# openjamoses/TOSEM-2021-Replication

Measured on NVIDIA H100. Metric: source MB/s scanned (tokenise + line-hash + classify + aggregate), higher is better.
Workload: dtype u8

## Files before the change

tosem-2021-replication_b200/csrc/tsm_device.cuh:

```cuda
#pragma once
#include <cstdint>
#include <cuda_runtime.h>
#include "../../include/tosemscan.h"
#include "../../include/tsm_categories.h"

namespace tsm {

constexpr uint32_t CH = 4096;
constexpr uint32_t PRE = 16;
constexpr uint32_t EXT = 240;
constexpr uint32_t BUF = PRE + CH + EXT;
constexpr uint32_t STRIPE = BUF / 32;
static_assert(STRIPE * 32 == BUF && STRIPE % 8 == 0 && (STRIPE / 8) % 2 == 1, "stripe geometry");
constexpr uint32_t LUT_BYTES = 1024 + 128;

constexpr uint32_t B_FIRST = (1u << 0) | (1u << 6) | (1u << 13) | (1u << 18) | (1u << 21) | (1u << 25) | (1u << 29) | (1u << 30) | (1u << 31);
constexpr uint32_t AF_ASSERT = 1u << 5, AF_EXPECT = 1u << 12, A_CLASS = 1u << 17, A_DEF = 1u << 20, A_TEST = 1u << 24,
                   A_VOID = 1u << 28, A_BRACE = 1u << 29, B_F = 1u << 30;
constexpr uint32_t PY_G1 = A_DEF, PY_G2 = A_CLASS, CJ_G1 = A_TEST, CJ_G2 = A_BRACE | A_CLASS | A_VOID;

constexpr uint8_t LF_CAND = 1, LF_HDR = 2, LF_FIX = 4;

struct Ctrl {
  uint32_t n_cand;
  uint32_t n_hev;
  uint32_t n_aev;
  uint32_t overflow;
  uint32_t n_lh;
  uint32_t lh_overflow;
  uint32_t cls_done;
};

constexpr unsigned long long TSM_DIFF_TRACE_MAX_INTS = 1ull << 28;
constexpr long long TSM_DIFF_TRACE_MAX_D = 23168;
static_assert((TSM_DIFF_TRACE_MAX_D + 1) * (TSM_DIFF_TRACE_MAX_D + 2) / 2 <= (long long)TSM_DIFF_TRACE_MAX_INTS && (TSM_DIFF_TRACE_MAX_D + 2) * (TSM_DIFF_TRACE_MAX_D + 3) / 2 > (long long)TSM_DIFF_TRACE_MAX_INTS, "cap");

struct SlabCtl { uint32_t n_units, work; };

struct ScanParams {
  const uint8_t* arena;
  const int32_t* off;
  const int32_t* len;
  const uint8_t* ext;
  const uint16_t* grp;
  int32_t n_files;
  int32_t n_groups;
  uint32_t* unit_file;
  uint32_t* unit_begin;
  uint32_t unit_cap;
  SlabCtl* slab;
  int32_t f_begin, f_end;
  uint32_t unit_base;
  Ctrl* ctrl;
  tsm_file_stat* stats;
  unsigned long long* cand;
  uint32_t cand_cap;
  tsm_header_event* hev;
  uint32_t hev_cap;
  tsm_assert_event* aev;
  uint32_t aev_cap;
  unsigned long long* counts;
  uint32_t flags;
  unsigned long long* lh_hash;
  uint32_t* lh_end;
  uint8_t* lh_flag;
  uint32_t lh_cap;
  uint32_t* unit_lines;
  uint32_t* unit_out;
  uint32_t four;
  uint32_t cls_last;
};

constexpr unsigned long long M61 = 0x1FFFFFFFFFFFFFFFull;

__device__ __forceinline__ unsigned long long fold61(unsigned long long x) { return (x & M61) + (x >> 61); }
__device__ __forceinline__ unsigned long long rotl61(unsigned long long x, uint32_t r) {
  return ((x << r) & M61) | (x >> (61 - r));
}
__device__ __forceinline__ unsigned long long canon61(unsigned long long acc) {
  acc = fold61(fold61(acc));
  return acc == M61 ? 0ull : acc;
}
__device__ __forceinline__ unsigned long long mix_hash(unsigned long long h61, unsigned long long len) {
  unsigned long long x = h61 ^ (len * 0x9E3779B97F4A7C15ull);
  x ^= x >> 30; x *= 0xBF58476D1CE4E5B9ull;
  x ^= x >> 27; x *= 0x94D049BB133111EBull;
  x ^= x >> 31;
  return x;
}

__device__ __forceinline__ bool is_w(uint32_t c) { return c == 0x20 || c == 0x09 || c == 0x0D || c == 0x0B || c == 0x0C; }
__device__ __forceinline__ bool is_ident(uint32_t c) {
  return (c - 'a') < 26u || (c - 'A') < 26u || (c - '0') < 10u || c == '_';
}

__device__ __forceinline__ uint32_t smem_u32(const void* p) { return (uint32_t)__cvta_generic_to_shared(p); }
__device__ __forceinline__ void mbar_init(uint64_t* bar, uint32_t count) {
  asm volatile("mbarrier.init.shared::cta.b64 [%0], %1;" ::"r"(smem_u32(bar)), "r"(count));
}
__device__ __forceinline__ void fence_mbar_init() { asm volatile("fence.mbarrier_init.release.cluster;" ::: "memory"); }
__device__ __forceinline__ void fence_proxy_async() { asm volatile("fence.proxy.async.shared::cta;" ::: "memory"); }
__device__ __forceinline__ void mbar_expect_tx(uint64_t* bar, uint32_t bytes) {
  asm volatile("mbarrier.arrive.expect_tx.shared::cta.b64 _, [%0], %1;" ::"r"(smem_u32(bar)), "r"(bytes) : "memory");
}
__device__ __forceinline__ void bulk_load(void* dst, const void* src, uint32_t bytes, uint64_t* bar) {
  asm volatile("cp.async.bulk.shared::cluster.global.mbarrier::complete_tx::bytes [%0], [%1], %2, [%3];"
               ::"r"(smem_u32(dst)), "l"(src), "r"(bytes), "r"(smem_u32(bar)) : "memory");
}
__device__ __forceinline__ bool mbar_try_wait(uint64_t* bar, uint32_t parity) {
  uint32_t ok;
  asm volatile("{\n\t.reg .pred p;\n\tmbarrier.try_wait.parity.shared::cta.b64 p, [%1], %2;\n\tselp.u32 %0, 1, 0, p;\n\t}"
               : "=r"(ok) : "r"(smem_u32(bar)), "r"(parity) : "memory");
  return ok != 0;
}

}
```

tosem-2021-replication_b200/csrc/tsm_scan_kernels.cuh:

```cuda
#pragma once
#include "tsm_device.cuh"

namespace tsm {

__constant__ uint32_t c_lut[256];
__constant__ uint32_t c_lut_b[256];
__constant__ uint32_t c_elut[256];
__device__ uint8_t c_cat_slot[TSM_CAT_SLOTS];
__device__ uint16_t c_cat_off[TSM_CAT_NAMED + 1];
__device__ char c_cat_blob[TSM_CAT_BLOB_LEN + 1];

__global__ void k_plan(ScanParams p) {
  const int f = p.f_begin + blockIdx.x * blockDim.x + threadIdx.x;
  const int lane = threadIdx.x & 31;
  if (blockIdx.x == 0 && threadIdx.x == 0) p.ctrl->cls_done = p.ctrl->n_cand;
  uint32_t nu = 0;
  if (f < p.f_end) {
    nu = ((uint32_t)p.len[f] + CH - 1) / CH;
    if (nu != 1) p.stats[f] = tsm_file_stat{0, 0, 0, 0, 0};
  }
  uint32_t incl = nu;
#pragma unroll
  for (int d = 1; d < 32; d <<= 1) {
    uint32_t t = __shfl_up_sync(0xffffffffu, incl, d);
    if (lane >= d) incl += t;
  }
  const uint32_t total = __shfl_sync(0xffffffffu, incl, 31);
  uint32_t base = 0;
  if (lane == 31 && total) base = atomicAdd(&p.slab->n_units, total);
  base = __shfl_sync(0xffffffffu, base, 31);
  uint32_t at = p.unit_base + base + incl - nu;
  for (uint32_t u = 0; u < nu; ++u, ++at) {
    if (at < p.unit_cap) { p.unit_file[at] = (uint32_t)f; p.unit_begin[at] = u * CH; }
    else p.ctrl->overflow = 1;
  }
}

__device__ __forceinline__ uint32_t nl_word(uint32_t w) {
  const uint32_t y = w ^ 0x0A0A0A0Au;
  const uint32_t t = (y & 0x7F7F7F7Fu) + 0x7F7F7F7Fu;
  const uint32_t z = ~(t | y | 0x7F7F7F7Fu);
  return (z * 0x00204081u) >> 28;
}
__device__ __forceinline__ uint32_t spaces_of(unsigned long long w) {
  const unsigned long long x = w ^ 0x2020202020202020ull, k7 = 0x7F7F7F7F7F7F7F7Full;
  const unsigned long long nz = (((x & k7) + k7) | x) & ~k7;
  return nz ? ((uint32_t)__ffsll((long long)nz) - 1u) >> 3 : 8u;
}
struct SmemByte {
  const uint8_t* b;
  __device__ __forceinline__ uint32_t operator()(uint32_t i) const { return b[i]; }
  __device__ __forceinline__ unsigned long long load8(uint32_t i) const {
    const uint32_t a = i & ~7u, sh = 8u * (i & 7u);
    const unsigned long long lo = *reinterpret_cast<const unsigned long long*>(b + a);
    const unsigned long long hi = *reinterpret_cast<const unsigned long long*>(b + a + 8);
    return sh ? (lo >> sh) | (hi << (64u - sh)) : lo;
  }
  __device__ __forceinline__ uint32_t spaces8(uint32_t i) const { return spaces_of(load8(i)); }
};
struct HbmByte {
  const uint8_t* b;
  __device__ __forceinline__ uint32_t operator()(uint32_t i) const { return __ldg(b + i); }
  __device__ __forceinline__ unsigned long long load8(uint32_t i) const {
    const unsigned long long* w = reinterpret_cast<const unsigned long long*>(b) + (i >> 3);
    const uint32_t sh = 8u * (i & 7u);
    const unsigned long long lo = __ldg(w), hi = __ldg(w + 1);
    return sh ? (lo >> sh) | (hi << (64u - sh)) : lo;
  }
  __device__ __forceinline__ uint32_t spaces8(uint32_t i) const { return spaces_of(load8(i)); }
};
struct Accum { uint32_t lines, asserts, hdrs, fixes; unsigned long long digest; };

__device__ __forceinline__ uint32_t warp_reserve(uint32_t* counter, uint32_t n, int lane) {
  uint32_t base = 0;
  if (lane == 0 && n) base = atomicAdd(counter, n);
  return __shfl_sync(0xffffffffu, base, 0);
}

__device__ __forceinline__ const uint32_t* scan_lut() {
  extern __shared__ __align__(128) uint8_t smem[];
  return reinterpret_cast<const uint32_t*>(smem);
}

__device__ __forceinline__ void issue_load(const ScanParams& p, uint8_t* buf, uint64_t* bar, uint32_t fo,
                                           uint32_t size, uint32_t cb) {
  const uint32_t lb = cb ? cb - PRE : 0u;
  const uint32_t le = min(cb + CH + EXT, size);
  const uint32_t bytes = (le - lb + 15u) & ~15u;
  mbar_expect_tx(bar, bytes);
  bulk_load(buf + PRE - (cb - lb), p.arena + (size_t)fo + lb, bytes, bar);
}

struct Unit { uint32_t u, f, cb, fo, size; int ext; };

__device__ __forceinline__ Unit claim_unit(const ScanParams& p, uint32_t n_units, int lane) {
  Unit x{0, 0, 0, 0, 0, 0};
  if (lane == 0) x.u = atomicAdd(&p.slab->work, 1u);
  x.u = __shfl_sync(0xffffffffu, x.u, 0);
  if (x.u < n_units) {
    x.f = p.unit_file[p.unit_base + x.u];
    x.cb = p.unit_begin[p.unit_base + x.u];
    x.fo = (uint32_t)p.off[x.f];
    x.size = (uint32_t)p.len[x.f];
    x.ext = p.ext[x.f];
  }
  return x;
}

constexpr uint32_t CC_W = 1, CC_IDENT = 2, CC_STOP = 4;
constexpr uint32_t CLS_CAT_OFF_N = (TSM_CAT_NAMED + 2) & ~1u;
constexpr uint32_t CLS_CAT_WORDS = ((TSM_CAT_SLOTS + 2 * CLS_CAT_OFF_N + TSM_CAT_BLOB_LEN + 15) / 16) * 4;
constexpr uint32_t CLS_SMEM_BASE = 4 * (512 + CLS_CAT_WORDS + 4 * 1024 + 4);
constexpr uint32_t E_FIRST = (1u << 0) | (1u << 5) | (1u << 9) | (1u << 17) | (1u << 21) | (1u << 23) | (1u << 25) |
                             (1u << 27) | (1u << 29) | (1u << 30);

struct FileBytes {
  const unsigned long long* base; uint32_t cur_blk; unsigned long long w;
  uint32_t blk0; unsigned long long w0, w1, w2, w3;
  __device__ __forceinline__ FileBytes(const uint8_t* b, uint32_t first_byte)
      : base(reinterpret_cast<const unsigned long long*>(b)), cur_blk(0xFFFFFFFFu), w(0), blk0(first_byte >> 3) {
    w0 = __ldg(base + blk0); w1 = __ldg(base + blk0 + 1); w2 = __ldg(base + blk0 + 2); w3 = __ldg(base + blk0 + 3);
  }
  __device__ __forceinline__ unsigned long long word(uint32_t blk) const {
    const uint32_t d = blk - blk0;
    if (d < 4u) return d < 2u ? (d == 0u ? w0 : w1) : (d == 2u ? w2 : w3);
    return __ldg(base + blk);
  }
  __device__ __forceinline__ uint32_t get(uint32_t i) {
    const uint32_t blk = i >> 3;
    if (blk != cur_blk) { w = word(blk); cur_blk = blk; }
    return (uint32_t)(w >> (8u * (i & 7u))) & 0xFFu;
  }
  __device__ __forceinline__ unsigned long long get8(uint32_t i) const {
    const uint32_t blk = i >> 3, sh = 8u * (i & 7u);
    const unsigned long long lo = word(blk);
    if (sh == 0) return lo;
    return (lo >> sh) | (word(blk + 1) << (64u - sh));
  }
};

__device__ __forceinline__ unsigned long long low_bytes(unsigned long long v, uint32_t n) {
  return n >= 8 ? v : (v & ((1ull << (8u * n)) - 1ull));
}

__device__ __forceinline__ int stem_lookup(FileBytes& rd, uint32_t s, uint32_t n) {
  if (n < 2 || n > 9) return 0;
  const unsigned long long v = low_bytes(rd.get8(s), n);
  const uint32_t c9 = n == 9 ? rd.get(s + 8) : 0u;
  switch (n) {
    case 2:
      if (v == 0x5145ull) return 1;
      if (v == 0x454Eull) return 2;
      if (v == 0x5447ull) return 5;
      if (v == 0x4547ull) return 6;
      if (v == 0x544Cull) return 7;
      if (v == 0x454Cull) return 8;
      return 0;
    case 4:
      if (v == 0x45555254ull) return 3;
      if (v == 0x5241454Eull) return 9;
      return 0;
    case 5:
      if (v == 0x45534C4146ull) return 4;
      if (v == 0x574F524854ull) return 12;
      return 0;
    case 8: return v == 0x51455F54414F4C46ull ? 10 : 0;
    case 9: return (v == 0x455F454C42554F44ull && c9 == 'Q') ? 11 : 0;
    default: return 0;
  }
}

__device__ __forceinline__ int bare_assert_category(FileBytes& rd, uint32_t e0, uint32_t en, const uint32_t* elut, int deflt = 3,
                                                    bool not_prefix = true) {
  if (not_prefix && en >= 4 && (uint32_t)rd.get8(e0) == 0x20746F6Eu) return 2;
  uint32_t D = 0, A = 0;
  for (uint32_t a = 0; a < en; a += 8) {
    unsigned long long w = rd.get8(e0 + a);
    if (en - a < 8) w &= (1ull << (8u * (en - a))) - 1ull;
    const uint32_t lo = (uint32_t)w, hi = (uint32_t)(w >> 32);
#pragma unroll
    for (int k = 0; k < 4; ++k) { D = ((D + D) | E_FIRST) & elut[__byte_perm(lo, 0, 0x4440 + k)]; A |= D; }
#pragma unroll
    for (int k = 0; k < 4; ++k) { D = ((D + D) | E_FIRST) & elut[__byte_perm(hi, 0, 0x4440 + k)]; A |= D; }
  }
  if (((A & (1u << 4)) && (A & (1u << 8))) || (A & (1u << 16))) return 4;
  if (A & (1u << 20)) return 3;
  if (A & (1u << 22)) return 1;
  if (A & (1u << 24)) return 2;
  if (A & (1u << 26)) return 8;
  if (A & (1u << 28)) return 6;
  if (A & (1u << 29)) return 7;
  if (A & (1u << 30)) return 5;
  return deflt;
}

__device__ __noinline__ bool ident_eq(FileBytes& rd, uint32_t s, uint32_t n, const char* name, uint32_t len) {
  if (n != len) return false;
  for (uint32_t k = 0; k < len; ++k)
    if (rd.get(s + k) != (uint8_t)name[k]) return false;
  return true;
}

constexpr uint32_t BQ_CAP = 1024;

#ifndef TSM_CLS_MINB
#define TSM_CLS_MINB 1
#endif
template <bool REVB>
__global__ void __launch_bounds__(256, TSM_CLS_MINB) k_classify_t(ScanParams p) {
  extern __shared__ __align__(16) uint32_t csm[];
  uint32_t* cls = csm;
  uint32_t* elut = csm + 256;
  uint8_t* cat_slot = reinterpret_cast<uint8_t*>(csm + 512);
  uint16_t* cat_off = reinterpret_cast<uint16_t*>(cat_slot + TSM_CAT_SLOTS);
  uint8_t* cat_blob = reinterpret_cast<uint8_t*>(cat_off + CLS_CAT_OFF_N);
  uint4* bq = reinterpret_cast<uint4*>(csm + 512 + CLS_CAT_WORDS);
  uint32_t* bqn = csm + 512 + CLS_CAT_WORDS + 4 * BQ_CAP;
  uint32_t* hist = bqn + 4;
  const bool use_smem = p.n_groups <= 16;
  for (int i = threadIdx.x; i < 256; i += blockDim.x) {
    const uint32_t c = (uint32_t)i;
    cls[i] = (is_w(c) ? CC_W : 0u) | (is_ident(c) ? CC_IDENT : 0u) | ((c == '(' || c == '\n') ? CC_STOP : 0u);
    elut[i] = c_elut[i];
  }
  for (int i = threadIdx.x; i < TSM_CAT_SLOTS; i += blockDim.x) cat_slot[i] = c_cat_slot[i];
  for (int i = threadIdx.x; i < TSM_CAT_NAMED + 1; i += blockDim.x) cat_off[i] = c_cat_off[i];
  for (int i = threadIdx.x; i < TSM_CAT_BLOB_LEN; i += blockDim.x) cat_blob[i] = (uint8_t)c_cat_blob[i];
  if (use_smem) for (int i = threadIdx.x; i < p.n_groups * TSM_K; i += blockDim.x) hist[i] = 0;
  if (threadIdx.x == 0) *bqn = 0;
  __syncthreads();
  auto count = [&](uint32_t f, int cat) {
    const uint32_t g = p.grp ? p.grp[f] : 0u;
    if (use_smem) atomicAdd(&hist[g * TSM_K + cat], 1u);
    else {
      atomicAdd(&p.counts[(size_t)g * TSM_K + cat], 1ull);
      atomicAdd(&p.counts[(size_t)p.n_groups * TSM_K + cat], 1ull);
    }
  };
  const uint32_t n = min(p.ctrl->n_cand, p.cand_cap), n0 = min(p.ctrl->cls_done, n);
  const bool want_ev = (p.flags & TSM_SCAN_ASSERT_EVENTS) != 0;
  constexpr bool revb = REVB;
  for (uint32_t i = n0 + blockIdx.x * blockDim.x + threadIdx.x; i < n; i += gridDim.x * blockDim.x) {
    const unsigned long long cd = p.cand[i];
    const uint32_t f = (uint32_t)(cd >> 32), line_off = (uint32_t)cd;
    const uint32_t size = (uint32_t)p.len[f];
    FileBytes rd(p.arena + (size_t)(uint32_t)p.off[f], line_off);
    uint32_t q = line_off;
    while (q < size && (cls[rd.get(q)] & CC_W)) ++q;
    const uint32_t t0 = q;
    uint32_t stop = size;
    for (uint32_t wb = t0 & ~7u; wb < size; wb += 8) {
      unsigned long long w = rd.word(wb >> 3);
      const unsigned long long x1 = w ^ 0x2828282828282828ull, x2 = w ^ 0x0A0A0A0A0A0A0A0Aull;
      const unsigned long long k7 = 0x7F7F7F7F7F7F7F7Full;
      unsigned long long z = (~(((x1 & k7) + k7) | x1 | k7)) | (~(((x2 & k7) + k7) | x2 | k7));
      if (wb < t0) z &= ~0ull << (8u * (t0 - wb));
      if (z) { stop = wb + ((uint32_t)__ffsll((long long)z) - 1u) / 8u; break; }
    }
    stop = min(stop, size);
    uint32_t last = stop;
    while (last > t0 && (cls[rd.get(last - 1)] & CC_W)) --last;
    uint32_t Ls = last;
    while (Ls > t0 && (cls[rd.get(Ls - 1)] & CC_IDENT)) --Ls;
    uint32_t tlen = last - t0;
    const uint32_t tlen_a = tlen, Ln = last - Ls;
    int cat = 0;
    bool done = false;
    uint32_t def_e0 = 0, def_en = 0;
    if (revb) {
      const bool macro = ident_eq(rd, Ls, Ln, "BOOST_CHECK", 11) || ident_eq(rd, Ls, Ln, "NTA_CHECK", 9);
      const bool bare6 = tlen == 6 && low_bytes(rd.get8(t0), 6) == 0x747265737361ull;
      const bool full = macro || p.ext[f] == TSM_EXT_JAVA;
      uint32_t fe = last;
      if (full || ((macro || bare6) && stop < size && rd.get(stop) == '(')) {
        uint32_t le = stop;
        while (le < size && rd.get(le) != '\n') ++le;
        fe = le;
        while (fe > t0 && (cls[rd.get(fe - 1)] & CC_W)) --fe;
      }
      if (ident_eq(rd, Ls, Ln, "BOOST_CHECK_EQUAL", 17)) { cat = 1; done = true; }
      else if ((macro || bare6) && stop < size && rd.get(stop) == '(') {
        uint32_t x = stop + 1;
        while (x < fe && (cls[rd.get(x)] & CC_W)) ++x;
        if (x < fe && rd.get(x) == '!' && !(x + 1 < fe && rd.get(x + 1) == '=')) cat = 4;
        else cat = bare_assert_category(rd, x, fe > x ? fe - x : 0u, elut, macro ? 0 : 3, false);
        done = true;
      }
      if (full) tlen = fe - t0;
    }
    if (Ln >= 7) {
      const unsigned long long h7 = low_bytes(rd.get8(Ls), 7);
      if (h7 == 0x5F544345505845ull || h7 == 0x5F545245535341ull) { cat = stem_lookup(rd, Ls + 7, Ln - 7); done = true; }
    }
    if (!done && tlen_a >= 6) {
      const unsigned long long h = rd.get8(t0);
      const bool a6 = low_bytes(h, 6) == 0x747265737361ull;
      if (a6 && tlen_a == 6) { cat = 3; done = true; }
      else if (a6 && tlen_a >= 8 && ((h >> 48) & 0xFF) == 0x20) {
        done = true;
        def_e0 = t0 + 7; def_en = tlen_a - 7;
      }
    }
    if (!done && Ln >= 6) {
      const unsigned long long h = rd.get8(Ls);
      if (low_bytes(h, 6) == 0x747265737361ull) {
        if (Ln == 7 && ((h >> 48) & 0xFF) == '_') cat = 3;
        else {
          cat = TSM_CAT_OTHER;
          uint32_t hh = 0x811C9DC5u;
          for (uint32_t j = 0; j < Ln; j += 8) {
            unsigned long long w = rd.get8(Ls + j);
            const uint32_t nb = min(8u, Ln - j);
#pragma unroll
            for (uint32_t k = 0; k < 8; ++k) {
              if (k < nb) hh = (hh ^ ((uint32_t)w & 0xFFu)) * 0x01000193u;
              w >>= 8;
            }
          }
          const int id = cat_slot[(hh * TSM_CAT_HASH_MULT) >> 23];
          if (id && (uint32_t)(cat_off[id + 1] - cat_off[id]) == Ln) {
            const uint8_t* name = cat_blob + cat_off[id];
            bool ok = true;
            for (uint32_t j = 0; j < Ln; j += 8) {
              unsigned long long w = rd.get8(Ls + j);
              const uint32_t nb = min(8u, Ln - j);
              for (uint32_t k = 0; k < nb; ++k) { ok &= ((uint32_t)w & 0xFFu) == (uint32_t)name[j + k]; w >>= 8; }
            }
            if (ok) cat = id;
          }
        }
      }
    }
    uint32_t ev_slot = 0xFFFFFFFFu;
    if (want_ev) {
      unsigned long long hacc = 0; uint32_t hr = 0;
      for (uint32_t j = 0; j < tlen; ++j) {
        hacc = fold61(hacc + rotl61((unsigned long long)rd.get(t0 + j), hr));
        hr += 8; if (hr >= 61) hr -= 61;
      }
      const uint32_t slot = atomicAdd(&p.ctrl->n_aev, 1u);
      if (slot < p.aev_cap) {
        tsm_assert_event ev;
        ev.file = f; ev.line_off = line_off; ev.stmt_off = t0;
        ev.stmt_len = (uint16_t)min(tlen, 65535u); ev.cat = (uint16_t)cat;
        ev.ident_off = Ls; ev.ident_len = (uint16_t)min(Ln, 65535u); ev.pad = 0;
        ev.stmt_hash = mix_hash(canon61(hacc), tlen);
        p.aev[slot] = ev;
        ev_slot = slot;
      } else p.ctrl->overflow = 1;
    }
    if (def_en) {
      const uint32_t slot = atomicAdd(bqn, 1u);
      if (slot < BQ_CAP) { bq[slot] = make_uint4(f, def_e0, def_en, ev_slot); continue; }
      cat = bare_assert_category(rd, def_e0, def_en, elut);
      if (ev_slot != 0xFFFFFFFFu) p.aev[ev_slot].cat = (uint16_t)cat;
    }
    count(f, cat);
  }
  __syncthreads();
  {
    const uint32_t nq = min(*bqn, BQ_CAP);
    for (uint32_t t = threadIdx.x; t < nq; t += blockDim.x) {
      const uint4 e = bq[t];
      FileBytes rd(p.arena + (size_t)(uint32_t)p.off[e.x], e.y);
      const int cat = bare_assert_category(rd, e.y, e.z, elut);
      if (e.w != 0xFFFFFFFFu) p.aev[e.w].cat = (uint16_t)cat;
      count(e.x, cat);
    }
  }
  if (p.cls_last) {
    unsigned long long t0 = 0, t1 = 0, t2 = 0, t3 = 0;
    for (int f = blockIdx.x * blockDim.x + threadIdx.x; f < p.n_files; f += gridDim.x * blockDim.x) {
      const tsm_file_stat s = p.stats[f];
      t0 += s.n_lines; t1 += s.n_assert; t2 += s.n_headers; t3 += s.n_fixture;
    }
#pragma unroll
    for (int d = 16; d; d >>= 1) {
      t0 += __shfl_xor_sync(0xffffffffu, t0, d); t1 += __shfl_xor_sync(0xffffffffu, t1, d);
      t2 += __shfl_xor_sync(0xffffffffu, t2, d); t3 += __shfl_xor_sync(0xffffffffu, t3, d);
    }
    if ((threadIdx.x & 31) == 0) {
      unsigned long long* tot = p.counts + (size_t)(p.n_groups + 1) * TSM_K;
      if (t0) atomicAdd(&tot[0], t0);
      if (t1) atomicAdd(&tot[1], t1);
      if (t2) atomicAdd(&tot[2], t2);
      if (t3) atomicAdd(&tot[3], t3);
    }
  }
  if (use_smem) {
    __syncthreads();
    for (int i = threadIdx.x; i < p.n_groups * TSM_K; i += blockDim.x) {
      const uint32_t v = hist[i];
      if (v) {
        atomicAdd(&p.counts[i], (unsigned long long)v);
        atomicAdd(&p.counts[(size_t)p.n_groups * TSM_K + (i & (TSM_K - 1))], (unsigned long long)v);
      }
    }
  }
}

template __global__ void k_classify_t<false>(ScanParams);
template __global__ void k_classify_t<true>(ScanParams);

}
```

tosem-2021-replication_b200/csrc/tsm_scan_walk.cuh:

```cuda
#pragma once
#include "tsm_scan_kernels.cuh"

namespace tsm {

#ifndef TSM_SCAN2_WARPS
#define TSM_SCAN2_WARPS 11
#endif
#ifndef TSM_SCAN2_CTAS
#define TSM_SCAN2_CTAS 2
#endif
#ifndef TSM_WALK_UNROLL
#define TSM_WALK_UNROLL 1
#endif
constexpr int SCAN2_WARPS = TSM_SCAN2_WARPS, SCAN2_CTAS_PER_SM = TSM_SCAN2_CTAS, WALK_UNROLL = TSM_WALK_UNROLL;

constexpr uint32_t NWORD = BUF / 8;
constexpr uint32_t O2_ARUN = BUF;
constexpr uint32_t SLOT_TAIL = NWORD;
constexpr uint32_t RW2_PER_STRIPE = 4;
constexpr uint32_t O2_RW = O2_ARUN + ((NWORD + 1) * 4 + 7) / 8 * 8;
constexpr uint32_t O2_WENT = O2_RW + 32 * RW2_PER_STRIPE * 8;
constexpr uint32_t WENT_CAP = NWORD + 8;
constexpr uint32_t LCAP = 512;
constexpr uint32_t O2_LTAB = O2_WENT + WENT_CAP * 2;
constexpr uint32_t O2_BASE = O2_LTAB + (LCAP + 8) * 2;
constexpr uint32_t Q2_CAP = 64;
constexpr uint32_t O2_Q = O2_BASE + 34 * 8;
constexpr uint32_t O2_CTL = O2_Q + Q2_CAP * 2;
constexpr uint32_t WARP_SMEM2 = ((O2_CTL + 16 + 127) / 128) * 128;
#ifndef TSM_PHASE_CLOCKS
#define TSM_PHASE_CLOCKS 0
#endif
enum ScanPhase { PH_WAIT, PH_ZERO, PH_WALK, PH_SCANS, PH_MIXED, PH_RECORDS, PH_FINISH, PH_LONG, PH_FLUSH, PH_N };
#if TSM_PHASE_CLOCKS
__device__ unsigned long long g_scan_phase_clk[PH_N];
#endif
struct PhaseClock {
#if TSM_PHASE_CLOCKS
  uint32_t* tab;
  long long t;
  __device__ __forceinline__ void mark(int ph, int lane) {
    const long long now = clock64();
    if (lane == 0) atomicAdd(tab + ph, (uint32_t)(now - t));
    t = now;
  }
#else
  __device__ __forceinline__ void mark(int, int) {}
#endif
};

constexpr uint32_t O2_T0A = LUT_BYTES;
constexpr uint32_t O2_PHASE = LUT_BYTES + 512;
constexpr uint32_t CTA_BYTES2 = LUT_BYTES + 512 + (TSM_PHASE_CLOCKS ? 128 : 0);
constexpr uint32_t SCAN2_SMEM = CTA_BYTES2 + SCAN2_WARPS * WARP_SMEM2;
constexpr uint32_t O2_LUTB = SCAN2_SMEM;
constexpr uint32_t SCAN2_SMEM_B = SCAN2_SMEM + 1024;
static_assert(O2_RW % 8 == 0 && O2_WENT % 8 == 0 && O2_LTAB % 2 == 0 && O2_BASE % 8 == 0 && O2_Q % 4 == 0 && O2_CTL % 8 == 0, "alignment");
static_assert(SCAN2_CTAS_PER_SM * (SCAN2_SMEM_B + 1024) <= 233472, "shared memory per SM (228 KB, 1 KB reserved per CTA)");
constexpr uint32_t LR_POS = 0x1FFFu, LR_FIRST = 0x2000u, LR_MIXED = 0x4000u, LR_VIRT = 0x8000u;

constexpr uint32_t B2_FIRST = (1u << 0) | (1u << 6) | (1u << 15), B2_FIN = (1u << 5) | (1u << 14) | (1u << 18);
constexpr uint32_t REVB_BIT = 1u;

struct LutRef { uint32_t four, base; };
__device__ __forceinline__ LutRef lut_ref() { return LutRef{scan_lut()[256 + 12], scan_lut()[256 + 13]}; }
template <bool REVB>
__device__ __forceinline__ void lut_at(uint32_t idx, LutRef t, uint32_t& v, uint32_t& v2) {
  uint32_t addr;
  asm("mad.lo.u32 %0, %1, %2, %3;" : "=r"(addr) : "r"(idx), "r"(t.four), "r"(t.base));
  asm("ld.shared.u32 %0, [%1];" : "=r"(v) : "r"(addr));
  if (REVB) asm("ld.shared.u32 %0, [%1+%2];" : "=r"(v2) : "r"(addr), "n"(O2_LUTB));
}

struct Auto { uint32_t D, D2; };

template <bool REVB>
__device__ __forceinline__ uint32_t step1(Auto& a, uint32_t byte, LutRef t) {
  uint32_t m, m2 = 0;
  lut_at<REVB>(byte, t, m, m2);
  a.D = ((a.D + a.D) | B_FIRST) & m;
  if (!REVB) return a.D;
  a.D2 = ((a.D2 + a.D2) | B2_FIRST) & m2;
  return (a.D & ~REVB_BIT) | ((a.D2 & B2_FIN) ? REVB_BIT : 0u);
}

template <bool REVB>
__device__ __forceinline__ void step8b(unsigned long long w, Auto& a, uint32_t& A, LutRef t) {
  const uint32_t lo = (uint32_t)w, hi = (uint32_t)(w >> 32);
  uint32_t A2 = 0;
#pragma unroll
  for (int k = 0; k < 8; ++k) {
    uint32_t m, m2 = 0;
    lut_at<REVB>(__byte_perm(k < 4 ? lo : hi, 0, 0x4440 + (k & 3)), t, m, m2);
    a.D = ((a.D + a.D) | B_FIRST) & m;
    A |= a.D;
    if (REVB) { a.D2 = ((a.D2 + a.D2) | B2_FIRST) & m2; A2 |= a.D2; }
  }
  if (REVB) A = (A & ~REVB_BIT) | ((A2 & B2_FIN) ? REVB_BIT : 0u);
}

__device__ __forceinline__ uint32_t nl8_of(unsigned long long w) {
  return nl_word((uint32_t)w) | (nl_word((uint32_t)(w >> 32)) << 4);
}
__device__ __forceinline__ unsigned long long low_mask(uint32_t b) {
  return b >= 8u ? ~0ull : ((1ull << (8u * b)) - 1ull);
}
__device__ __forceinline__ unsigned long long ror3_61(unsigned long long r) { return (r >> 3) + ((r & 7ull) << 58); }

struct WalkOut { uint32_t nlw, tail; };

template <bool REVB>
__device__ __noinline__ WalkOut walk2(uint8_t* wb, uint32_t fin, int lane) {
  const uint32_t pos0 = (uint32_t)lane * STRIPE;
  const uint8_t* sp = wb + pos0;
  uint32_t* ar = reinterpret_cast<uint32_t*>(wb + O2_ARUN) + (uint32_t)lane * 17u;
  unsigned long long* rw = reinterpret_cast<unsigned long long*>(wb + O2_RW) + (uint32_t)lane * RW2_PER_STRIPE;
  const LutRef t = lut_ref();
  Auto au{0u, 0u};
  if (lane) {
    uint32_t A = 0;
    step8b<REVB>(*reinterpret_cast<const unsigned long long*>(sp - 8), au, A, t);
  }
  unsigned long long R = 0;
  uint32_t run = 0, nlr = 0;
  auto word = [&](uint32_t k) {
    const unsigned long long w = *reinterpret_cast<const unsigned long long*>(sp + 8u * k);
    uint32_t A = 0;
    step8b<REVB>(w, au, A, t);
    R = ror3_61(R) + fold61(w);
    ar[k] = run;
    nlr = __funnelshift_l(A, nlr, 1);
    const bool nl = (int32_t)A < 0;
    if (nl && (A & fin)) {
      const uint32_t slot = atomicAdd(reinterpret_cast<uint32_t*>(wb + O2_CTL), 1u);
      if (slot < Q2_CAP) reinterpret_cast<uint16_t*>(wb + O2_Q)[slot] = (uint16_t)((uint32_t)lane * 17u + k);
    }
    run = nl ? 0u : (run | A);
  };
#pragma unroll 1
  for (uint32_t g = 0; g < 4; ++g) {
#pragma unroll WALK_UNROLL
    for (uint32_t k = 0; k < 4; ++k) word(4u * g + k);
    rw[g] = R;
  }
  word(16);
  unsigned long long incl = rotl61(canon61(R), (3u * (17u * (uint32_t)lane + 16u)) % 61u);
#pragma unroll
  for (int d = 1; d < 32; d <<= 1) {
    const unsigned long long t = __shfl_up_sync(0xffffffffu, incl, d);
    if (lane >= d) incl = fold61(incl + t);
  }
  unsigned long long excl = __shfl_up_sync(0xffffffffu, incl, 1);
  if (lane == 0) excl = 0;
  unsigned long long* sbase = reinterpret_cast<unsigned long long*>(wb + O2_BASE);
  sbase[lane] = excl;
  if (lane == 31) sbase[32] = incl;
  return WalkOut{__brev(nlr) >> 15, run};
}

template <bool REVB>
__device__ __noinline__ void resolve_mixed(uint8_t* wb, uint32_t g, uint32_t i, uint32_t n_went) {
  const LutRef t = lut_ref();
  Auto au{0u, 0u};
  uint32_t A = 0;
  step8b<REVB>(*reinterpret_cast<const unsigned long long*>(wb + 8u * g - 8u), au, A, t);
  unsigned long long w = *reinterpret_cast<const unsigned long long*>(wb + 8u * g);
  uint32_t pre = 0, post = 0, seen = 0;
#pragma unroll
  for (int b = 0; b < 8; ++b) {
    const uint32_t d = step1<REVB>(au, (uint32_t)w & 0xFFu, t);
    const uint32_t m = (uint32_t)((int32_t)au.D >> 31);
    pre |= d & ~seen;
    seen |= m;
    post = (post | d) & ~m;
    w >>= 8;
  }
  uint32_t* arun = reinterpret_cast<uint32_t*>(wb + O2_ARUN);
  const uint16_t* went = reinterpret_cast<const uint16_t*>(wb + O2_WENT);
  atomicOr(arun + g, pre);
  const uint32_t tgt = i + 1u < n_went ? ((uint32_t)went[i + 1u] & 0x3FFu) : SLOT_TAIL;
  atomicOr(arun + tgt, post);
}

__device__ __forceinline__ void emit_header(const ScanParams& p, uint32_t f, uint32_t line_off, uint32_t len, uint32_t fl) {
  const uint32_t slot = atomicAdd(&p.ctrl->n_hev, 1u);
  if (slot < p.hev_cap) p.hev[slot] = tsm_header_event{f, line_off, len, (fl >> 2) & 1u};
  else p.ctrl->overflow = 1;
}

template <typename Bytes>
__device__ __noinline__ bool starts_with8(Bytes lb, uint32_t s, uint32_t e, unsigned long long pat, uint32_t n, bool need_ws) {
  uint32_t r;
  while (s + 8 <= e && (r = lb.spaces8(s)) != 0) { s += r; if (r < 8) break; }
  while (s < e && is_w(lb(s))) ++s;
  if (s + n + (need_ws ? 1u : 0u) > e) return false;
  const unsigned long long v = lb.load8(s);
  if ((v & low_mask(n)) != pat) return false;
  if (need_ws) {
    const uint32_t c = (uint32_t)(v >> (8u * n)) & 0xFFu;
    if (c != 0x20 && c != 0x09) return false;
    for (uint32_t q = s + n + 1; q < e; ++q)
      if (!is_w(lb(q))) return true;
    return false;
  }
  return true;
}

template <bool REVB, typename Bytes>
__device__ __forceinline__ uint32_t line_flags2(uint32_t s, uint32_t e, uint32_t A, uint32_t g1, uint32_t g2, int ext, Bytes lb, Accum& ac) {
  if (ext == 0) return 0;
  uint32_t fl = (A & (AF_ASSERT | AF_EXPECT | (REVB ? REVB_BIT : 0u))) ? LF_CAND : 0;
  bool hdr;
  if (ext == TSM_EXT_PY) {
    hdr = (A & g1) != 0;
    if (!hdr && (A & g2)) hdr = starts_with8(lb, s, e, 0x7373616C63ull, 5, true);
  } else {
    hdr = (A & g1) != 0 && (A & g2) != 0;
  }
  if (hdr) { fl |= LF_HDR; if ((A & B_F) && starts_with8(lb, s, e, 0x465F54534554ull, 6, false)) fl |= LF_FIX; }
  ac.asserts += fl & LF_CAND;
  ac.hdrs += (fl >> 1) & 1u;
  ac.fixes += (fl >> 2) & 1u;
  return fl;
}

struct FinishState {
  Accum ac;
  uint32_t prev_last;
  unsigned long long prevP;
  uint32_t lh_base, lh_done;
};

template <bool REVB>
__device__ __noinline__ FinishState finish_lines2(const ScanParams& p, uint8_t* wb, const uint32_t* lc, uint32_t n, uint32_t lim,
                                                  bool skip_first, uint32_t f, uint32_t cb, int ext, int lane, FinishState fs) {
  uint16_t* ltab = reinterpret_cast<uint16_t*>(wb + O2_LTAB);
  const uint32_t* arun = reinterpret_cast<const uint32_t*>(wb + O2_ARUN);
  const unsigned long long* t0a = reinterpret_cast<const unsigned long long*>(scan_lut()) + O2_T0A / 8;
  const uint32_t g1 = lc[1], g2 = lc[2];
  const SmemByte lb{wb};
  const bool want_hev = (p.flags & TSM_SCAN_HEADER_EVENTS) != 0, want_lh = (p.flags & TSM_SCAN_LINE_HASHES) != 0;
  Accum a = fs.ac;
  uint32_t nc = 0, lh_done = fs.lh_done;
  uint32_t prev_last = fs.prev_last;
  unsigned long long prevP = fs.prevP;
  for (uint32_t base = 0; base < n; base += 32) {
    const uint32_t j = base + (uint32_t)lane;
    const bool valid = j < n;
    const uint32_t rec = valid ? (uint32_t)ltab[j] : 0u;
    const uint32_t e = rec & LR_POS;
    const bool isv = (rec & LR_VIRT) != 0;
    const uint32_t g = min(e >> 3, NWORD - 1u), b1 = e - 8u * g + (isv ? 0u : 1u);
    const uint32_t l = g / 17u, i = g - 17u * l, c0 = i >> 2, ns = i & 3u;
    unsigned long long R = 0;
    if (c0) R = *reinterpret_cast<const unsigned long long*>(wb + O2_RW + 8u * (l * RW2_PER_STRIPE + c0 - 1u));
    const unsigned long long* wp = reinterpret_cast<const unsigned long long*>(wb) + (g - ns);
#pragma unroll
    for (uint32_t t = 0; t < 3u; ++t)
      if (ns > t) R = ror3_61(R) + fold61(wp[t]);
    const unsigned long long w = *reinterpret_cast<const unsigned long long*>(wb + 8u * g);
    const uint32_t r3g = (3u * g) % 61u;
    const unsigned long long X = ror3_61(R) + fold61(w & low_mask(b1));
    unsigned long long Pn = *reinterpret_cast<const unsigned long long*>(wb + O2_BASE + 8u * l) + rotl61(fold61(fold61(X)), r3g);
    uint32_t r8e = r3g + 8u * (e & 7u);
    if (r8e >= 61u) r8e -= 61u;
    const unsigned long long Pe = isv ? Pn : Pn + M61 - t0a[r8e];
    uint32_t s = __shfl_up_sync(0xffffffffu, e, 1) + 1u;
    unsigned long long Ps = __shfl_up_sync(0xffffffffu, Pn, 1);
    if (lane == 0) { s = prev_last + 1u; Ps = prevP; }
    const int src = base + 32u <= n ? 31 : (int)(n - 1u - base);
    prev_last = __shfl_sync(0xffffffffu, e, src);
    prevP = __shfl_sync(0xffffffffu, Pn, src);
    const bool owned = valid && s < lim && !(s == PRE && skip_first);
    uint32_t fl = 0;
    unsigned long long lh = 0;
    if (owned) {
      const unsigned long long hr = canon61(Pe + 4ull * M61 - Ps);
      const uint32_t sh = (8u * s) % 61u;
      unsigned long long h = rotl61(hr, sh ? 61u - sh : 0u);
      uint32_t len = e - s;
      if (len && lb(e - 1u) == 0x0D) {
        --len;
        const unsigned long long cr = rotl61(0x0Dull, (8u * len) % 61u);
        h = h >= cr ? h - cr : h + M61 - cr;
      }
      a.lines++;
      lh = mix_hash(h, len);
      a.digest += lh;
      uint32_t A = 0;
      if (rec & LR_FIRST) A = arun[isv ? SLOT_TAIL : g];
      else if (rec & LR_MIXED) {
        Auto au{0u, 0u};
        const LutRef t = lut_ref();
        for (uint32_t q = s; q < e; ++q) A |= step1<REVB>(au, lb(q), t);
      }
      fl = line_flags2<REVB>(s, e, A, g1, g2, ext, lb, a);
      if (want_hev && (fl & LF_HDR)) emit_header(p, f, cb + s - PRE, e - s, fl);
    }
    if (want_lh) {
      const uint32_t mo = __ballot_sync(0xffffffffu, owned);
      const uint32_t slot = fs.lh_base + lh_done + __popc(mo & ((1u << lane) - 1u));
      if (owned && slot < p.lh_cap) {
        p.lh_hash[slot] = lh;
        p.lh_end[slot] = cb + e - PRE;
        p.lh_flag[slot] = (uint8_t)(fl & LF_CAND);
      }
      lh_done += __popc(mo);
    }
    __syncwarp();
    const uint32_t mc = __ballot_sync(0xffffffffu, fl & LF_CAND);
    if (fl & LF_CAND) ltab[nc + __popc(mc & ((1u << lane) - 1u))] = (uint16_t)s;
    nc += __popc(mc);
  }
  __syncwarp();
  if (nc && p.cand_cap) {
    const uint32_t cbase = warp_reserve(&p.ctrl->n_cand, nc, lane);
    for (uint32_t i = (uint32_t)lane; i < nc; i += 32) {
      const uint32_t slot = cbase + i;
      if (slot < p.cand_cap) p.cand[slot] = ((unsigned long long)f << 32) | (cb + (uint32_t)ltab[i] - PRE);
      else p.ctrl->overflow = 1;
    }
  }
  __syncwarp();
  fs.ac = a;
  fs.prev_last = prev_last;
  fs.prevP = prevP;
  fs.lh_done = lh_done;
  return fs;
}

template <bool REVB>
__device__ __noinline__ Accum long_line(const ScanParams& p, const uint32_t* lc, uint32_t f, uint32_t size, int ext,
                                        uint32_t s, uint32_t lh_slot, Accum ac) {
  const HbmByte lb{p.arena + (uint32_t)p.off[f]};
  uint32_t e = s;
  while (e < size && lb(e) != '\n') ++e;
  const uint32_t k0 = s >> 3, k1 = (e - 1u) >> 3;
  const LutRef t = lut_ref();
  Auto au{0u, 0u};
  uint32_t A = 0;
  unsigned long long R = 0;
#pragma unroll 1
  for (uint32_t k = k0; k <= k1; ++k) {
    unsigned long long w = __ldg(reinterpret_cast<const unsigned long long*>(lb.b) + k);
    if (k == k0) w &= ~0ull << (8u * (s & 7u));
    if (k == k1) w &= low_mask(e - 8u * k);
    uint32_t Aw = 0;
    step8b<REVB>(w, au, Aw, t);
    A |= Aw;
    R = ror3_61(R) + fold61(w);
  }
  unsigned long long h = rotl61(canon61(R), (3u * (k1 - k0) + 61u * 8u - 8u * (s & 7u)) % 61u);
  uint32_t len = e - s;
  if (lb(e - 1u) == 0x0D) {
    --len;
    const unsigned long long cr = rotl61(0x0Dull, (8u * len) % 61u);
    h = h >= cr ? h - cr : h + M61 - cr;
  }
  const unsigned long long lh = mix_hash(h, len);
  ac.lines++;
  ac.digest += lh;
  const uint32_t fl = line_flags2<REVB>(s, e, A, lc[1], lc[2], ext, lb, ac);
  if ((fl & LF_CAND) && p.cand_cap) {
    const uint32_t slot = atomicAdd(&p.ctrl->n_cand, 1u);
    if (slot < p.cand_cap) p.cand[slot] = ((unsigned long long)f << 32) | s;
    else p.ctrl->overflow = 1;
  }
  if ((fl & LF_HDR) && (p.flags & TSM_SCAN_HEADER_EVENTS)) emit_header(p, f, s, e - s, fl);
  if ((p.flags & TSM_SCAN_LINE_HASHES) && lh_slot < p.lh_cap) {
    p.lh_hash[lh_slot] = lh;
    p.lh_end[lh_slot] = e;
    p.lh_flag[lh_slot] = (uint8_t)(fl & LF_CAND);
  }
  return ac;
}

template <bool REVB>
__device__ __forceinline__ void process_chunk2(const ScanParams& p, const uint32_t* lc, uint8_t* wb, uint32_t uslot, uint32_t f,
                                               uint32_t cb, uint32_t size, int ext, int lane, PhaseClock& pc) {
  const uint32_t ce = min(cb + CH, size);
  const uint32_t le = min(ce + EXT, size);
  const uint32_t lim = PRE + (ce - cb);
  const uint32_t lim2 = PRE + (le - cb);
  const bool skip_first = (cb != 0) && (wb[PRE - 1] != '\n');
  __syncwarp();
  if (lane < 2) reinterpret_cast<unsigned long long*>(wb)[lane] = 0ull;
  {
    const uint32_t za = (lim2 + 7u) & ~7u;
    if ((uint32_t)lane < za - lim2) wb[lim2 + lane] = 0;
    for (uint32_t q = za + 8u * (uint32_t)lane; q < BUF; q += 256u) *reinterpret_cast<unsigned long long*>(wb + q) = 0ull;
  }
  if (lane == 0) *reinterpret_cast<uint32_t*>(wb + O2_CTL) = 0u;
  __syncwarp();
  pc.mark(PH_ZERO, lane);
  const WalkOut wo = walk2<REVB>(wb, lc[0], lane);
  pc.mark(PH_WALK, lane);
  const uint32_t w0 = 17u * (uint32_t)lane, lim_w = (lim + 7u) >> 3;
  const uint32_t ownbits = lim_w <= w0 ? 0u : (lim_w - w0 >= 17u ? 0x1FFFFu : (1u << (lim_w - w0)) - 1u);
  const uint32_t extbits = wo.nlw & ~ownbits;
  const uint32_t gx = __reduce_min_sync(0xffffffffu, extbits ? w0 + (uint32_t)__ffs((int)extbits) - 1u : 0xFFFFu);
  uint32_t kept = wo.nlw & ownbits;
  if (gx - w0 < 17u) kept |= 1u << (gx - w0);
  uint32_t tv = wo.tail, tf = wo.nlw != 0u;
  const uint32_t cnt = __popc(kept);
  uint32_t incl = cnt;
#pragma unroll
  for (int d = 1; d < 32; d <<= 1) {
    const uint32_t uv = __shfl_up_sync(0xffffffffu, tv, d), uf = __shfl_up_sync(0xffffffffu, tf, d);
    const uint32_t t = __shfl_up_sync(0xffffffffu, incl, d);
    if (lane >= d) { if (!tf) tv |= uv; tf |= uf; incl += t; }
// ... 191 lines not shown
```

Measured before the change: 614,800.

## Add SWAR register-window fast path for assert classification with deferred long-path queue

The classify kernel now loads a 64-byte window per candidate line into registers and uses SWAR byte tests to find the statement start, stop, and identifier bounds. It then matches categories and computes the statement hash without byte-by-byte FileBytes reads. Lines that don't fit the window, or that hit special cases, go into a shared-memory queue and run through the original slow path after a block barrier. This cuts divergent serial byte loops, but adds register pressure, which is partly offset by raising min-blocks in the launch bounds. The change also carries risk of subtle mismatches against the original semantics.

```diff
diff --git a/tosem-2021-replication_b200/csrc/tsm_device.cuh b/tosem-2021-replication_b200/csrc/tsm_device.cuh
--- a/tosem-2021-replication_b200/csrc/tsm_device.cuh
+++ b/tosem-2021-replication_b200/csrc/tsm_device.cuh
@@ -77,6 +77,7 @@
 __device__ __forceinline__ unsigned long long rotl61(unsigned long long x, uint32_t r) {
   return ((x << r) & M61) | (x >> (61 - r));
 }
+__device__ __forceinline__ unsigned long long ror3_61(unsigned long long r) { return (r >> 3) + ((r & 7ull) << 58); }
 __device__ __forceinline__ unsigned long long canon61(unsigned long long acc) {
   acc = fold61(fold61(acc));
   return acc == M61 ? 0ull : acc;
diff --git a/tosem-2021-replication_b200/csrc/tsm_scan_kernels.cuh b/tosem-2021-replication_b200/csrc/tsm_scan_kernels.cuh
--- a/tosem-2021-replication_b200/csrc/tsm_scan_kernels.cuh
+++ b/tosem-2021-replication_b200/csrc/tsm_scan_kernels.cuh
@@ -110,7 +110,7 @@
 constexpr uint32_t CC_W = 1, CC_IDENT = 2, CC_STOP = 4;
 constexpr uint32_t CLS_CAT_OFF_N = (TSM_CAT_NAMED + 2) & ~1u;
 constexpr uint32_t CLS_CAT_WORDS = ((TSM_CAT_SLOTS + 2 * CLS_CAT_OFF_N + TSM_CAT_BLOB_LEN + 15) / 16) * 4;
-constexpr uint32_t CLS_SMEM_BASE = 4 * (512 + CLS_CAT_WORDS + 4 * 1024 + 4);
+constexpr uint32_t CLS_SMEM_BASE = 4 * (512 + CLS_CAT_WORDS + 4 * 1024 + 4 + 256);
 constexpr uint32_t E_FIRST = (1u << 0) | (1u << 5) | (1u << 9) | (1u << 17) | (1u << 21) | (1u << 23) | (1u << 25) |
                              (1u << 27) | (1u << 29) | (1u << 30);
 
@@ -143,10 +143,9 @@
   return n >= 8 ? v : (v & ((1ull << (8u * n)) - 1ull));
 }
 
-__device__ __forceinline__ int stem_lookup(FileBytes& rd, uint32_t s, uint32_t n) {
+__device__ __forceinline__ int stem_lookup(unsigned long long s8, uint32_t c9, uint32_t n) {
   if (n < 2 || n > 9) return 0;
-  const unsigned long long v = low_bytes(rd.get8(s), n);
-  const uint32_t c9 = n == 9 ? rd.get(s + 8) : 0u;
+  const unsigned long long v = low_bytes(s8, n);
   switch (n) {
     case 2:
       if (v == 0x5145ull) return 1;
@@ -202,9 +201,43 @@
 }
 
 constexpr uint32_t BQ_CAP = 1024;
+constexpr uint32_t LQ_CAP = 256;
+static_assert(CLS_SMEM_BASE == 4 * (512 + CLS_CAT_WORDS + 4 * BQ_CAP + 4 + LQ_CAP), "k_classify shared-memory layout");
+
+constexpr uint32_t WIN = 64;
+constexpr uint32_t cat_name_max() {
+  constexpr uint16_t off[TSM_CAT_NAMED + 1] = TSM_CAT_OFF_INIT;
+  uint32_t m = 0;
+  for (int i = 0; i < TSM_CAT_NAMED; ++i) m = (uint32_t)(off[i + 1] - off[i]) > m ? (uint32_t)(off[i + 1] - off[i]) : m;
+  return m;
+}
+constexpr uint32_t CAT_NAME_MAX = cat_name_max();
+static_assert(CAT_NAME_MAX >= 17 && CAT_NAME_MAX / 4 + 1 <= 16, "k_classify reads L's bytes up to the longest name (and 17 for Rev B)");
+__device__ __forceinline__ uint32_t nib4(uint32_t z) { return (z * 0x00204081u) >> 28; }
+
+template <int NO>
+__device__ __forceinline__ void win_at(const uint32_t (&x)[16], uint32_t r, uint32_t (&out)[NO]) {
+  uint32_t a[16];
+#pragma unroll
+  for (int j = 0; j < 16; ++j) a[j] = x[j];
+#pragma unroll
+  for (int st = 8; st >= 1; st >>= 1) {
+    const bool on = (r & (4u * st)) != 0;
+#pragma unroll
+    for (int j = 0; j < 16; ++j) a[j] = on ? (j + st < 16 ? a[j + st] : 0u) : a[j];
+  }
+  const uint32_t sh = 8u * (r & 3u);
+#pragma unroll
+  for (int k = 0; k < NO; ++k) out[k] = __funnelshift_r(a[k], k + 1 < 16 ? a[k + 1] : 0u, sh);
+}
+__device__ __forceinline__ unsigned long long u64_of(uint32_t lo, uint32_t hi) { return ((unsigned long long)hi << 32) | lo; }
+__device__ __forceinline__ unsigned long long low_mask64(uint32_t n) { return n >= 64u ? ~0ull : (1ull << n) - 1ull; }
+__host__ __device__ constexpr unsigned long long le_bytes(const char* s, int n) {
+  return n == 0 ? 0ull : (unsigned long long)(uint8_t)s[0] | (le_bytes(s + 1, n - 1) << 8);
+}
 
 #ifndef TSM_CLS_MINB
-#define TSM_CLS_MINB 1
+#define TSM_CLS_MINB 4
 #endif
 template <bool REVB>
 __global__ void __launch_bounds__(256, TSM_CLS_MINB) k_classify_t(ScanParams p) {
@@ -216,7 +249,8 @@
   uint8_t* cat_blob = reinterpret_cast<uint8_t*>(cat_off + CLS_CAT_OFF_N);
   uint4* bq = reinterpret_cast<uint4*>(csm + 512 + CLS_CAT_WORDS);
   uint32_t* bqn = csm + 512 + CLS_CAT_WORDS + 4 * BQ_CAP;
-  uint32_t* hist = bqn + 4;
+  uint32_t* lq = bqn + 4;
+  uint32_t* hist = lq + LQ_CAP;
   const bool use_smem = p.n_groups <= 16;
   for (int i = threadIdx.x; i < 256; i += blockDim.x) {
     const uint32_t c = (uint32_t)i;
@@ -227,7 +261,7 @@
   for (int i = threadIdx.x; i < TSM_CAT_NAMED + 1; i += blockDim.x) cat_off[i] = c_cat_off[i];
   for (int i = threadIdx.x; i < TSM_CAT_BLOB_LEN; i += blockDim.x) cat_blob[i] = (uint8_t)c_cat_blob[i];
   if (use_smem) for (int i = threadIdx.x; i < p.n_groups * TSM_K; i += blockDim.x) hist[i] = 0;
-  if (threadIdx.x == 0) *bqn = 0;
+  if (threadIdx.x == 0) { bqn[0] = 0; bqn[1] = 0; }
   __syncthreads();
   auto count = [&](uint32_t f, int cat) {
     const uint32_t g = p.grp ? p.grp[f] : 0u;
@@ -240,7 +274,31 @@
   const uint32_t n = min(p.ctrl->n_cand, p.cand_cap), n0 = min(p.ctrl->cls_done, n);
   const bool want_ev = (p.flags & TSM_SCAN_ASSERT_EVENTS) != 0;
   constexpr bool revb = REVB;
-  for (uint32_t i = n0 + blockIdx.x * blockDim.x + threadIdx.x; i < n; i += gridDim.x * blockDim.x) {
+  auto finish = [&](uint32_t f, uint32_t line_off, uint32_t t0, uint32_t tlen, uint32_t Ls, uint32_t Ln, int cat,
+                    unsigned long long h61, uint32_t def_e0, uint32_t def_en) {
+    uint32_t ev_slot = 0xFFFFFFFFu;
+    if (want_ev) {
+      const uint32_t slot = atomicAdd(&p.ctrl->n_aev, 1u);
+      if (slot < p.aev_cap) {
+        tsm_assert_event ev;
+        ev.file = f; ev.line_off = line_off; ev.stmt_off = t0;
+        ev.stmt_len = (uint16_t)min(tlen, 65535u); ev.cat = (uint16_t)cat;
+        ev.ident_off = Ls; ev.ident_len = (uint16_t)min(Ln, 65535u); ev.pad = 0;
+        ev.stmt_hash = mix_hash(h61, tlen);
+        p.aev[slot] = ev;
+        ev_slot = slot;
+      } else p.ctrl->overflow = 1;
+    }
+    if (def_en) {
+      const uint32_t slot = atomicAdd(bqn, 1u);
+      if (slot < BQ_CAP) { bq[slot] = make_uint4(f, def_e0, def_en, ev_slot); return; }
+      FileBytes rd(p.arena + (size_t)(uint32_t)p.off[f], def_e0);
+      cat = bare_assert_category(rd, def_e0, def_en, elut);
+      if (ev_slot != 0xFFFFFFFFu) p.aev[ev_slot].cat = (uint16_t)cat;
+    }
+    count(f, cat);
+  };
+  auto long_path = [&](uint32_t i) {
     const unsigned long long cd = p.cand[i];
     const uint32_t f = (uint32_t)(cd >> 32), line_off = (uint32_t)cd;
     const uint32_t size = (uint32_t)p.len[f];
@@ -290,7 +348,7 @@
     }
     if (Ln >= 7) {
       const unsigned long long h7 = low_bytes(rd.get8(Ls), 7);
-      if (h7 == 0x5F544345505845ull || h7 == 0x5F545245535341ull) { cat = stem_lookup(rd, Ls + 7, Ln - 7); done = true; }
+      if (h7 == 0x5F544345505845ull || h7 == 0x5F545245535341ull) { cat = stem_lookup(rd.get8(Ls + 7), rd.get(Ls + 15), Ln - 7); done = true; }
     }
     if (!done && tlen_a >= 6) {
       const unsigned long long h = rd.get8(t0);
@@ -331,32 +389,138 @@
         }
       }
     }
-    uint32_t ev_slot = 0xFFFFFFFFu;
+    unsigned long long hacc = 0;
     if (want_ev) {
-      unsigned long long hacc = 0; uint32_t hr = 0;
+      uint32_t hr = 0;
       for (uint32_t j = 0; j < tlen; ++j) {
         hacc = fold61(hacc + rotl61((unsigned long long)rd.get(t0 + j), hr));
         hr += 8; if (hr >= 61) hr -= 61;
       }
-      const uint32_t slot = atomicAdd(&p.ctrl->n_aev, 1u);
-      if (slot < p.aev_cap) {
-        tsm_assert_event ev;
-        ev.file = f; ev.line_off = line_off; ev.stmt_off = t0;
-        ev.stmt_len = (uint16_t)min(tlen, 65535u); ev.cat = (uint16_t)cat;
-        ev.ident_off = Ls; ev.ident_len = (uint16_t)min(Ln, 65535u); ev.pad = 0;
-        ev.stmt_hash = mix_hash(canon61(hacc), tlen);
-        p.aev[slot] = ev;
-        ev_slot = slot;
-      } else p.ctrl->overflow = 1;
-    }
-    if (def_en) {
-      const uint32_t slot = atomicAdd(bqn, 1u);
-      if (slot < BQ_CAP) { bq[slot] = make_uint4(f, def_e0, def_en, ev_slot); continue; }
-      cat = bare_assert_category(rd, def_e0, def_en, elut);
-      if (ev_slot != 0xFFFFFFFFu) p.aev[ev_slot].cat = (uint16_t)cat;
-    }
-    count(f, cat);
-  }
+    }
+    finish(f, line_off, t0, tlen, Ls, Ln, cat, canon61(hacc), def_e0, def_en);
+  };
+  auto to_long_path = [&](uint32_t i) {
+    const uint32_t slot = atomicAdd(&bqn[1], 1u);
+    if (slot < LQ_CAP) lq[slot] = i;
+    else long_path(i);
+  };
+  for (uint32_t i = n0 + blockIdx.x * blockDim.x + threadIdx.x; i < n; i += gridDim.x * blockDim.x) {
+    const unsigned long long cd = p.cand[i];
+    const uint32_t f = (uint32_t)(cd >> 32), line_off = (uint32_t)cd;
+    const uint32_t lim = (uint32_t)p.len[f] - line_off;
+    uint32_t x[16];
+    {
+      const unsigned long long* fw =
+          reinterpret_cast<const unsigned long long*>(p.arena + (size_t)(uint32_t)p.off[f]) + (line_off >> 3);
+      uint32_t h[18];
+#pragma unroll
+      for (int k = 0; k < 9; ++k) { const unsigned long long v = __ldg(fw + k); h[2 * k] = (uint32_t)v; h[2 * k + 1] = (uint32_t)(v >> 32); }
+      const bool o4 = (line_off & 4u) != 0;
+      const uint32_t sh = 8u * (line_off & 3u);
+#pragma unroll
+      for (int j = 0; j < 16; ++j) x[j] = __funnelshift_r(o4 ? h[j + 1] : h[j], o4 ? h[j + 2] : h[j + 1], sh);
+    }
+    if (lim < WIN) {
+#pragma unroll
+      for (int j = 0; j < 16; ++j) {
+        const uint32_t v = lim > 4u * j ? lim - 4u * j : 0u;
+        if (v < 4u) x[j] &= (1u << (8u * v)) - 1u;
+      }
+    }
+    unsigned long long nbm = 0, stm = 0, nim = 0, pam = 0;
+#pragma unroll
+    for (int j = 0; j < 16; ++j) {
+      const uint32_t v = x[j], k7 = 0x7F7F7F7Fu, M = 0x80808080u, ascii = ~v & M, a = v & k7;
+      const uint32_t t_lf = ((v ^ 0x0A0A0A0Au) & k7) + k7, t_pa = ((v ^ 0x28282828u) & k7) + k7;
+      const uint32_t t_sp = ((v ^ 0x20202020u) & k7) + k7, t_us = ((v ^ 0x5F5F5F5Fu) & k7) + k7;
+      const uint32_t blank = (((a + 0x77777777u) & ~(a + 0x72727272u) & t_lf) | ~t_sp) & ascii;
+      const uint32_t lc = (v | 0x20202020u) & k7;
+      const uint32_t ident = (((((lc + 0x1F1F1F1Fu) & ~(lc + 0x05050505u)) | ~(a + 0x46464646u)) & (a + 0x50505050u)) | ~t_us) & ascii;
+      nbm |= (unsigned long long)nib4(~blank & M) << (4 * j);
+      stm |= (unsigned long long)nib4(~(t_lf & t_pa) & ascii) << (4 * j);
+      nim |= (unsigned long long)nib4(~ident & M) << (4 * j);
+      if (revb) pam |= (unsigned long long)nib4(~t_pa & ascii) << (4 * j);
+    }
+    const uint32_t t0r = nbm ? (uint32_t)__ffsll((long long)nbm) - 1u : WIN;
+    const unsigned long long sfrom = stm & ~low_mask64(t0r);
+    if (nbm == 0 || (sfrom == 0 && lim > WIN)) { to_long_path(i); continue; }
+    const uint32_t stopr = sfrom ? (uint32_t)__ffsll((long long)sfrom) - 1u : lim;
+    const unsigned long long nbs = nbm & low_mask64(stopr);
+    const uint32_t lastr = nbs ? 64u - (uint32_t)__clzll((long long)nbs) : t0r;
+    const unsigned long long nil = nim & low_mask64(lastr);
+    const uint32_t Lsr = max(nil ? 64u - (uint32_t)__clzll((long long)nil) : 0u, t0r);
+    const uint32_t tlen = lastr - t0r, Ln = lastr - Lsr;
+    uint32_t lw[CAT_NAME_MAX / 4 + 1], tw[2];
+    win_at(x, Lsr, lw);
+    win_at(x, t0r, tw);
+    const unsigned long long L0 = u64_of(lw[0], lw[1]), L1 = u64_of(lw[2], lw[3]), T8 = u64_of(tw[0], tw[1]);
+    int cat = 0;
+    bool done = false;
+    uint32_t def_e0 = 0, def_en = 0;
+    if (revb) {
+      const bool macro = (Ln == 11 && L0 == le_bytes("BOOST_CH", 8) && low_bytes(L1, 3) == le_bytes("ECK", 3)) ||
+                         (Ln == 9 && L0 == le_bytes("NTA_CHEC", 8) && (L1 & 0xFFu) == 'K');
+      const bool bare6 = tlen == 6 && low_bytes(T8, 6) == 0x747265737361ull;
+      if (macro || p.ext[f] == TSM_EXT_JAVA || (bare6 && stopr < WIN && ((pam >> stopr) & 1u))) { to_long_path(i); continue; }
+      if (Ln == 17 && L0 == le_bytes("BOOST_CH", 8) && L1 == le_bytes("ECK_EQUA", 8) && (lw[4] & 0xFFu) == 'L') { cat = 1; done = true; }
+    }
+    if (Ln >= 7) {
+      const unsigned long long h7 = low_bytes(L0, 7);
+      if (h7 == 0x5F544345505845ull || h7 == 0x5F545245535341ull) {
+        cat = stem_lookup((L0 >> 56) | (L1 << 8), (uint32_t)(L1 >> 56), Ln - 7); done = true;
+      }
+    }
+    if (!done && tlen >= 6) {
+      const bool a6 = low_bytes(T8, 6) == 0x747265737361ull;
+      if (a6 && tlen == 6) { cat = 3; done = true; }
+      else if (a6 && tlen >= 8 && ((T8 >> 48) & 0xFF) == 0x20) { done = true; def_e0 = line_off + t0r + 7; def_en = tlen - 7; }
+    }
+    if (!done && Ln >= 6 && low_bytes(L0, 6) == 0x747265737361ull) {
+      if (Ln == 7 && ((L0 >> 48) & 0xFF) == '_') cat = 3;
+      else {
+        cat = TSM_CAT_OTHER;
+        if (Ln <= CAT_NAME_MAX) {
+          uint32_t hh = 0x811C9DC5u;
+#pragma unroll
+          for (uint32_t j = 0; j < CAT_NAME_MAX / 4 + 1; ++j) {
+            if (4u * j < Ln) {
+#pragma unroll
+              for (uint32_t k = 0; k < 4; ++k)
+                if (4u * j + k < Ln) hh = (hh ^ ((lw[j] >> (8u * k)) & 0xFFu)) * 0x01000193u;
+            }
+          }
+          const int id = cat_slot[(hh * TSM_CAT_HASH_MULT) >> 23];
+          if (id && (uint32_t)(cat_off[id + 1] - cat_off[id]) == Ln) {
+            const uint8_t* name = cat_blob + cat_off[id];
+            bool ok = true;
+#pragma unroll
+            for (uint32_t j = 0; j < CAT_NAME_MAX / 4 + 1; ++j) {
+              if (4u * j < Ln) {
+#pragma unroll
+                for (uint32_t k = 0; k < 4; ++k)
+                  if (4u * j + k < Ln) ok &= ((lw[j] >> (8u * k)) & 0xFFu) == (uint32_t)name[4u * j + k];
+              }
+            }
+            if (ok) cat = id;
+          }
+        }
+      }
+    }
+    unsigned long long h61 = 0;
+    if (want_ev) {
+      unsigned long long R = 0;
+#pragma unroll
+      for (uint32_t k = 0; k < 8; ++k) {
+        const uint32_t b0 = t0r > 8u * k ? min(t0r - 8u * k, 8u) : 0u, b1 = lastr > 8u * k ? min(lastr - 8u * k, 8u) : 0u;
+        const unsigned long long m = low_bytes(~0ull, b1) & ~low_bytes(~0ull, b0);
+        R = ror3_61(R) + fold61(u64_of(x[2 * k], x[2 * k + 1]) & m);
+      }
+      h61 = rotl61(canon61(R), (21u + 61u * 9u - 8u * t0r) % 61u);
+    }
+    finish(f, line_off, line_off + t0r, tlen, line_off + Lsr, Ln, cat, h61, def_e0, def_en);
+  }
+  __syncthreads();
+  for (uint32_t t = threadIdx.x; t < min(bqn[1], LQ_CAP); t += blockDim.x) long_path(lq[t]);
   __syncthreads();
   {
     const uint32_t nq = min(*bqn, BQ_CAP);
diff --git a/tosem-2021-replication_b200/csrc/tsm_scan_walk.cuh b/tosem-2021-replication_b200/csrc/tsm_scan_walk.cuh
--- a/tosem-2021-replication_b200/csrc/tsm_scan_walk.cuh
+++ b/tosem-2021-replication_b200/csrc/tsm_scan_walk.cuh
@@ -105,7 +105,6 @@
 __device__ __forceinline__ unsigned long long low_mask(uint32_t b) {
   return b >= 8u ? ~0ull : ((1ull << (8u * b)) - 1ull);
 }
-__device__ __forceinline__ unsigned long long ror3_61(unsigned long long r) { return (r >> 3) + ((r & 7ull) << 58); }
 
 struct WalkOut { uint32_t nlw, tail; };
 
```

Result: faster. 624,800 (median of 6 runs) (+1.6%).
